# gudbrandtandberg/ChessVision-3LC

Hardware: AMD Instinct MI355X
Metric: boards/sec (UNet 256x256 seg + 64-sq classify) (higher is better)
Workload: dtype f16x3; 1 GPU; e2e-cnn b=256/GPU: UNet(3->1,convT) 256x256 x256 boards + ResNet-18(1ch,13cls) x16384 squares/step; in HBM (configs[3]); boards_per_gpu=256, parallelism=replicas x1, boards sharded, weights RCCL-broadcast once

## Files before the change

chessvision-3lc_amd/csrc/conv_device.h:

```cpp
#pragma once
#include <type_traits>

#include "cv_kernels.h"

namespace cv {

#ifndef CV_STAMP
#define CV_STAMP 0
#endif
#ifndef CV_IGEMM_PIPE
#define CV_IGEMM_PIPE 1
#endif
#ifndef CV_SCHED_HINTS
#define CV_SCHED_HINTS 1
#endif
#ifndef CV_SETPRIO
#define CV_SETPRIO 1
#endif
constexpr bool kSetPrio = CV_SETPRIO != 0;
#ifndef CV_ABLATE
#define CV_ABLATE 0
#endif

template <typename T> struct FragT;
template <> struct FragT<half_t> { typedef half8 V; };
template <> struct FragT<float>  { typedef f4 V; };
template <> struct FragT<split_t> { typedef half8 V; };

__device__ __forceinline__ void mma16(f4& acc, const half8& a, const half8& b) {
#if CV_ABLATE == 2
    asm volatile("" ::"v"(a), "v"(b));
#else
    acc = __builtin_amdgcn_mfma_f32_16x16x32_f16(a, b, acc, 0, 0, 0);
#endif
}
__device__ __forceinline__ void mma16(f4& acc, const f4& a, const f4& b) {
    acc = __builtin_amdgcn_mfma_f32_16x16x4f32(a[0], b[0], acc, 0, 0, 0);
    acc = __builtin_amdgcn_mfma_f32_16x16x4f32(a[1], b[1], acc, 0, 0, 0);
    acc = __builtin_amdgcn_mfma_f32_16x16x4f32(a[2], b[2], acc, 0, 0, 0);
    acc = __builtin_amdgcn_mfma_f32_16x16x4f32(a[3], b[3], acc, 0, 0, 0);
}

__device__ __forceinline__ void glds16(const char* g, char* l) {
    __builtin_amdgcn_global_load_lds((const __attribute__((address_space(1))) void*)g,
                                     (__attribute__((address_space(3))) void*)l, 16, 0, 0);
}

__device__ __forceinline__ void glds16s(const char* sbase, unsigned voff, char* l) {
    __builtin_amdgcn_global_load_lds((const __attribute__((address_space(1))) void*)(sbase + voff),
                                     (__attribute__((address_space(3))) void*)l, 16, 0, 0);
}

template <int N> __device__ __forceinline__ void wait_vm_barrier() {
    asm volatile("s_waitcnt vmcnt(%0) lgkmcnt(0)\n\ts_barrier" ::"n"(N) : "memory");
}

template <typename T, int N> struct OutVec;
template <int N> struct OutVec<half_t, N> {
    static __device__ __forceinline__ void store(half_t* dst, int, const float* v, float& bad) {
#pragma unroll
        for (int i = 0; i < N; i += 8) {
            half8 h;
#pragma unroll
            for (int j = 0; j < 8; ++j) { h[j] = (half_t)v[i + j]; bad = __builtin_fmaf((float)h[j], 0.f, bad); }
            *reinterpret_cast<half8*>(dst + i) = h;
        }
    }
    static constexpr int kRawChunks = N / 8;
    static __device__ __forceinline__ void fetch(const half_t* src, f4* raw) {
#pragma unroll
        for (int i = 0; i < N / 8; ++i) raw[i] = *reinterpret_cast<const f4*>(src + i * 8);
    }
    static __device__ __forceinline__ void add_raw(const f4* raw, int, float* v, float mul) {
#pragma unroll
        for (int i = 0; i < N; i += 8) {
            const half8 h = __builtin_bit_cast(half8, raw[i / 8]);
#pragma unroll
            for (int j = 0; j < 8; ++j) v[i + j] = __builtin_fmaf((float)h[j], mul, v[i + j]);
        }
    }
    static __device__ __forceinline__ void add(const half_t* src, int, float* v, float mul) {
#pragma unroll
        for (int i = 0; i < N; i += 8) {
            const half8 h = *reinterpret_cast<const half8*>(src + i);
#pragma unroll
            for (int j = 0; j < 8; ++j) v[i + j] = __builtin_fmaf((float)h[j], mul, v[i + j]);
        }
    }
};
template <int N> struct OutVec<float, N> {
    static __device__ __forceinline__ void store(float* dst, int, const float* v, float& bad) {
#pragma unroll
        for (int i = 0; i < N; i += 4) {
            f4 o = {v[i], v[i + 1], v[i + 2], v[i + 3]};
#pragma unroll
            for (int j = 0; j < 4; ++j) bad = __builtin_fmaf(o[j], 0.f, bad);
            *reinterpret_cast<f4*>(dst + i) = o;
        }
    }
    static constexpr int kRawChunks = N / 4;
    static __device__ __forceinline__ void fetch(const float* src, f4* raw) {
#pragma unroll
        for (int i = 0; i < N / 4; ++i) raw[i] = *reinterpret_cast<const f4*>(src + i * 4);
    }
    static __device__ __forceinline__ void add_raw(const f4* raw, int, float* v, float) {
#pragma unroll
        for (int i = 0; i < N; i += 4) { v[i] += raw[i / 4][0]; v[i + 1] += raw[i / 4][1]; v[i + 2] += raw[i / 4][2]; v[i + 3] += raw[i / 4][3]; }
    }
    static __device__ __forceinline__ void add(const float* src, int, float* v, float) {
#pragma unroll
        for (int i = 0; i < N; i += 4) {
            const f4 o = *reinterpret_cast<const f4*>(src + i);
            v[i] += o[0]; v[i + 1] += o[1]; v[i + 2] += o[2]; v[i + 3] += o[3];
        }
    }
};
template <int N> struct OutVec<split_t, N> {
    static __device__ __forceinline__ void store(split_t* dst, int ch0, const float* v, float& bad) {
        char* p = reinterpret_cast<char*>(dst);
#pragma unroll
        for (int i = 0; i < N; i += 8) {
            const int par = ((ch0 + i) >> 3) & 1;
            typedef _Float16 h2 __attribute__((ext_vector_type(2)));
            typedef unsigned u4 __attribute__((ext_vector_type(4)));
            u4 hu, lu;
            h2 g2 = {(half_t)0.f, (half_t)0.f};
#pragma unroll
            for (int j = 0; j < 8; j += 2) {
                unsigned hp, lp;
                split_pair(v[i + j], v[i + j + 1], hp, lp);
                g2 = __builtin_elementwise_fma(__builtin_bit_cast(h2, hp), h2{(half_t)0.f, (half_t)0.f}, g2);
                hu[j / 2] = hp; lu[j / 2] = lp;
            }
// ... 65 lines not shown
```

chessvision-3lc_amd/csrc/conv_halo.hip:

```cpp
#include "cv_kernels.h"
#include "conv_igemm.h"
#include "conv_device.h"

#include <cstdlib>

namespace cv {

constexpr int kHaloCT = 64, kHaloNW = 4, kHaloNSW = 3;
constexpr int halo_waves_per_eu(int chain) { return chain == 1 ? 1 : 2; }
template <typename T, int TH, int IMG, bool PERSIST, bool FUSE0 = false, int CHAIN = 0, int CNB = 2>
__global__ __launch_bounds__(64 * kHaloNW) __attribute__((amdgpu_waves_per_eu(halo_waves_per_eu(CHAIN), halo_waves_per_eu(CHAIN)))) void conv3x3_halo_kernel(const ConvParams p) {
    constexpr int CT = kHaloCT, NW = kHaloNW, NSW = kHaloNSW;
    constexpr bool DBH = TH == 8;
    static_assert(CT == 64 && NSW == 3, "every wave owns a 64-channel slab; the ring slot of a stage is tap % 3");
    static_assert(TH == 16 || (TH == 8 && IMG == 0 && !PERSIST), "16 x 16 patch with one halo buffer | 8 x 16 patch, double buffered");
    static_assert(!FUSE0 || (!DBH && !PERSIST && IMG == 0 && __is_same(T, split_t)), "fused producer: split-f16 64-channel single-halo tile");
    static_assert(!CHAIN || (!DBH && !PERSIST && !FUSE0 && IMG == 0 && __is_same(T, half_t)), "chained convolutions: f16 64-channel single-halo tile over whole 16 x 16 images");
    static_assert(CNB == 2 || (CHAIN && CNB == 3), "two or three chained BasicBlocks");
    constexpr int SPC = 9;
    constexpr int FC = 4;
    constexpr int FP = TH / NW;
    static_assert(FP >= 1 && FP <= 4 && TH % NW == 0, "wave tile");
    constexpr int WSTAGE = CT * 128;
    static_assert(IMG == 0 || (IMG == 8 && TH == 16), "packed-image mode: 2 x 2 images of 8 x 8");
    constexpr int HLW = IMG ? IMG + 2 : 18;
    constexpr int HR = IMG ? 4 * HLW * HLW : 18 * (TH + 2);
    constexpr int H = ((HR + 7) / 8 + NW - 1) / NW;
    constexpr int HBYTES = H * NW * 1024;
    constexpr int LW = CT / (8 * NW);
    static_assert(LW >= 1 && LW + H <= 63, "vmcnt range");
    constexpr bool kSplit16 = sizeof(T) == 4 && !__is_same(T, float);
    typedef typename FragT<T>::V V;

    extern __shared__ __attribute__((aligned(16))) char smem[];
    char* const halo = smem + NSW * WSTAGE;
#if CV_STAMP
    const unsigned long long st_k0 = __builtin_amdgcn_s_memtime();
#endif

    const int tid = threadIdx.x;
    const int lane = tid & 63;
    const int wave = __builtin_amdgcn_readfirstlane(tid >> 6);
    const unsigned nwg = gridDim.x, bid = blockIdx.x;
    const unsigned xq = nwg >> 3, xr = nwg & 7, xcd = bid & 7;
    const unsigned lid = (xcd < xr ? xcd * (xq + 1) : xr * (xq + 1) + (xcd - xr) * xq) + (bid >> 3);
    const int tilesX = IMG ? 1 : p.Wo / 16, tilesY = IMG ? 1 : p.Ho / TH;
    const int nImg = p.M / (p.Ho * p.Wo);
    const int kSplits = (!PERSIST && !FUSE0 && IMG == 0 && p.ksplit > 1) ? p.ksplit : 1;
    const int nCbAll = p.nStages / 9;
    int nCb = nCbAll, nS = nCb * SPC, cbBase = 0, ksCur = 0;
    const unsigned nTiles = (unsigned)((IMG ? (nImg + 3) / 4 : nImg * tilesX * tilesY) * p.nCt);
    int ctTile, tx, ty, n;
    unsigned hbase;
    const char* wsrc;
    unsigned hoff[H];

    const unsigned xpix = (unsigned)p.xCs * (unsigned)sizeof(T);
    const char* const xsrc = p.x + p.xCoffBytes;
    const int wi = wave;
    const unsigned lane16 = (unsigned)lane * 16u;
    auto halo_row_offset = [&](int i) __attribute__((always_inline)) -> unsigned {
        const int r = (i * NW + wi) * 8 + (lane >> 3);
        const int rr = r < HR ? r : HR - 1;
        if constexpr (IMG == 0) {
            const int hy = rr / 18, hx = rr - hy * 18;
            return (hbase + (unsigned)(hy * p.xWp + hx)) * xpix + (unsigned)(((lane & 7) ^ (hx & 7)) * 16);
        } else {
            const int lim = (nImg - n) * (HLW * HLW) - 1;
            const int rc = rr < lim ? rr : lim;
            const int hx = (rr % (HLW * HLW)) % HLW;
            return (unsigned)(n * (HLW * HLW) + rc) * xpix + (unsigned)(((lane & 7) ^ (hx & 7)) * 16);
        }
    };
    auto decode = [&](unsigned tile) __attribute__((always_inline)) {
        int pt;
        if (kSplits > 1) {
            const int nPatch = nImg * tilesX * tilesY;
            pt = tile % nPatch;
            const int rest = tile / nPatch;
            ctTile = rest % p.nCt;
            ksCur = rest / p.nCt;
            cbBase = ksCur * p.kper;
            nCb = nCbAll - cbBase < p.kper ? nCbAll - cbBase : p.kper;
            nS = nCb * SPC;
        } else {
            ctTile = tile % p.nCt;
            pt = tile / p.nCt;
        }
        tx = pt % tilesX; pt /= tilesX;
        ty = pt % tilesY;
        n = IMG ? 4 * (pt / tilesY) : pt / tilesY;
        hbase = (unsigned)((n * p.xHp + ty * TH) * p.xWp + tx * 16);
        wsrc = p.w + ((size_t)ctTile * p.nStages + (size_t)cbBase * 9) * WSTAGE + wi * 1024;
#pragma unroll
        for (int i = 0; i < H; ++i) hoff[i] = halo_row_offset(i);
    };

    const int q = lane >> 4, l15 = lane & 15;
    auto issue_w = [&](int s, int slot) __attribute__((always_inline)) {
        char* sW = smem + slot * WSTAGE;
#pragma unroll
        for (int i = 0; i < LW; ++i) glds16s(wsrc + (size_t)s * WSTAGE + i * (NW * 1024), lane16, sW + (i * NW + wi) * 1024);
    };
    auto issue_halo = [&](int cb, int hb) __attribute__((always_inline)) {
        char* sH = halo + hb * HBYTES;
        const char* const src = xsrc + (cbBase + cb) * 128;
#pragma unroll
        for (int i = 0; i < H; ++i) glds16s(src, hoff[i], sH + (i * NW + wi) * 1024);
    };

    constexpr int PW0 = 20;
    unsigned* const patch0 = reinterpret_cast<unsigned*>(halo + HBYTES);
    half8* const w0lds = reinterpret_cast<half8*>(halo + HBYTES + 4864);
    float* const sc0lds = reinterpret_cast<float*>(halo + HBYTES + 4864 + 4096);
    auto load_patch0 = [&]() __attribute__((always_inline)) {
        w0lds[tid] = reinterpret_cast<const half8*>(p.f0_w)[2 * 2 * 64 + tid];
        if (tid < 64) { sc0lds[tid] = p.f0_scale[tid]; sc0lds[64 + tid] = p.f0_shift[tid]; }
        float bad0 = 0.f;
        for (int idx = tid; idx < 3 * 20 * PW0 + 1; idx += 64 * NW) {
            const int c = idx / (20 * PW0), rem = idx - c * (20 * PW0), r = rem / PW0, col = rem - r * PW0;
            const int gy = ty * TH - 2 + r, gx = tx * 16 - 2 + col;
            float v = 0.f;
            if (idx < 3 * 20 * PW0 && gy >= 0 && gy < p.xHp - 2 && gx >= 0 && gx < p.xWp - 2) {
                const int Hh = p.xHp - 2, Ww = p.xWp - 2;
                if (p.f0_u8) v = (float)reinterpret_cast<const uint8_t*>(p.f0_x)[((size_t)(n * Hh + gy) * Ww + gx) * 3 + c] / 255.f;
                else v = reinterpret_cast<const float*>(p.f0_x)[((size_t)(n * 3 + c) * Hh + gy) * Ww + gx];
            }
            bad0 = __builtin_fmaf(v, 0.f, bad0);
            v *= p.f0_in_mul;
            const half_t vh = (half_t)v;
            const half_t vl = (half_t)(v - (float)vh);
            patch0[idx] = (unsigned)__builtin_bit_cast(unsigned short, vh) | ((unsigned)__builtin_bit_cast(unsigned short, vl) << 16);
        }
        if (bad0 != bad0 && p.flag) atomicMin(p.flag, 0u);
    };
    auto produce0 = [&](int cb) __attribute__((always_inline)) {
        half8 ah0, al0, ah1, al1;
        if (cb == 0) {
            const half8* w0 = reinterpret_cast<const half8*>(p.f0_w) + lane;
            ah0 = w0[0 * 64]; al0 = w0[1 * 64]; ah1 = w0[2 * 64]; al1 = w0[3 * 64];
        } else {
            ah0 = w0lds[0 * 64 + lane]; al0 = w0lds[1 * 64 + lane]; ah1 = w0lds[2 * 64 + lane]; al1 = w0lds[3 * 64 + lane];
        }
        float sc0[8], sh0[8];
#pragma unroll
        for (int j = 0; j < 8; j += 4) {
            const f4 a = *reinterpret_cast<const f4*>(sc0lds + cb * 32 + q * 8 + j);
            const f4 b = *reinterpret_cast<const f4*>(sc0lds + 64 + cb * 32 + q * 8 + j);
            sc0[j] = a[0]; sc0[j + 1] = a[1]; sc0[j + 2] = a[2]; sc0[j + 3] = a[3];
            sh0[j] = b[0]; sh0[j + 1] = b[1]; sh0[j + 2] = b[2]; sh0[j + 3] = b[3];
        }
        int ko[8];
#pragma unroll
        for (int j = 0; j < 8; ++j) {
            const int k = q * 8 + j, tap = k / 3, c = k - tap * 3, ky = tap / 3, kx = tap - ky * 3;
            ko[j] = k < 27 ? (c * 20 + ky) * PW0 + kx : 3 * 20 * PW0;
        }
        constexpr int NF = (HR + 15) / 16, U = 3;
        typedef unsigned u4 __attribute__((ext_vector_type(4)));
        int hp = wave * 16 + l15;
        int hy = hp / 18, hx = hp - hy * 18;
        for (int fr0 = wave; fr0 < NF; fr0 += U * NW) {
            int hyu[U], hxu[U], hpu[U];
            unsigned w8[U][8];
#pragma unroll
            for (int u = 0; u < U; ++u) {
                hpu[u] = hp;
                const bool tail = hp >= HR;
                hyu[u] = tail ? 17 : hy; hxu[u] = tail ? 17 : hx;
                const int pb = hyu[u] * PW0 + hxu[u];
#pragma unroll
                for (int j = 0; j < 8; ++j) w8[u][j] = patch0[(q * 8 + j < 27 ? pb : 0) + ko[j]];
                hp += 16 * NW;
                hx += (16 * NW) % 18; hy += (16 * NW) / 18;
                if (hx >= 18) { hx -= 18; hy += 1; }
            }
            f4 a0[U], a1[U];
            half8 bh[U], bl[U];
#pragma unroll
            for (int u = 0; u < U; ++u) {
                u4 uh, ul;
#pragma unroll
                for (int m = 0; m < 4; ++m) {
                    uh[m] = __builtin_amdgcn_perm(w8[u][2 * m + 1], w8[u][2 * m], 0x05040100u);
                    ul[m] = __builtin_amdgcn_perm(w8[u][2 * m + 1], w8[u][2 * m], 0x07060302u);
                }
                bh[u] = __builtin_bit_cast(half8, uh); bl[u] = __builtin_bit_cast(half8, ul);
            }
#pragma unroll
            for (int u = 0; u < U; ++u) {
                a0[u] = __builtin_amdgcn_mfma_f32_16x16x32_f16(ah0, bh[u], f4{0.f, 0.f, 0.f, 0.f}, 0, 0, 0);
                a1[u] = __builtin_amdgcn_mfma_f32_16x16x32_f16(ah1, bh[u], f4{0.f, 0.f, 0.f, 0.f}, 0, 0, 0);
            }
#pragma unroll
            for (int u = 0; u < U; ++u) {
                a0[u] = __builtin_amdgcn_mfma_f32_16x16x32_f16(al0, bh[u], a0[u], 0, 0, 0);
                a1[u] = __builtin_amdgcn_mfma_f32_16x16x32_f16(al1, bh[u], a1[u], 0, 0, 0);
// ... 108 lines not shown
#pragma unroll
                for (int f = 0; f < 4; ++f) rtrunk[g][f] = *reinterpret_cast<const f4*>(rb + (size_t)(pix0 + (unsigned)(g * p.yWp)) * 64 + f * 4);
        }
    };
    auto chain_epilogue = [&](int c) __attribute__((always_inline)) {
        if constexpr (CHAIN) {
            const bool has_res = (c & 1) != 0, last = c == 2 * CNB - 1;
            const int blk = c >> 1;
            const float* const scp = p.ch_scale[c] + q * 16;
            const float* const shp = p.ch_shift[c] + q * 16;
            float sc[16], sh[16];
#pragma unroll
            for (int i = 0; i < 16; i += 4) {
                const f4 a = *reinterpret_cast<const f4*>(scp + i);
                const f4 b = *reinterpret_cast<const f4*>(shp + i);
                sc[i] = a[0]; sc[i + 1] = a[1]; sc[i + 2] = a[2]; sc[i + 3] = a[3];
                sh[i] = b[0]; sh[i + 1] = b[1]; sh[i + 2] = b[2]; sh[i + 3] = b[3];
            }
            const unsigned pix0 = (unsigned)((n * p.yHp + wrow0 + 1) * p.yWp + l15 + 1);
            f4 r[2][4];
            const float* const rb = reinterpret_cast<const float*>(blk == 0 ? p.ch_res0 : p.ch_y32_mid[blk - 1]) + q * 16;
            auto fetch_res = [&](int g) __attribute__((always_inline)) {
#pragma unroll
                for (int f = 0; f < 4; ++f) r[g & 1][f] = *reinterpret_cast<const f4*>(rb + (size_t)(pix0 + (unsigned)(g * p.yWp)) * 64 + f * 4);
            };
            if (CHAIN == 2 && has_res) fetch_res(0);
            const float rm = p.ch_res_mul[blk];
            float* const o32 = reinterpret_cast<float*>(has_res && !last ? p.ch_y32_mid[blk] : p.y32) + q * 16;
            half_t* const o16 = reinterpret_cast<half_t*>(p.y) + q * 16;
            const int hx = l15 + 1;
            float bad = 0.f;
#pragma unroll
            for (int g = 0; g < FP; ++g) {
                if (CHAIN == 2 && has_res && g + 1 < FP) fetch_res(g + 1);
                float v[16];
#pragma unroll
                for (int f = 0; f < 4; ++f)
#pragma unroll
                    for (int k = 0; k < 4; ++k) {
                        float t = acc[f][g][k] * sc[f * 4 + k] + sh[f * 4 + k];
                        if constexpr (CHAIN == 2) {
                            if (has_res) t = __builtin_fmaf(r[g & 1][f][k], rm, t);
                        } else {
                            if (has_res) t = __builtin_fmaf(rtrunk[g][f][k], rm, t);
                        }
                        v[f * 4 + k] = __builtin_fmaxf(t, 0.f);
                        if constexpr (CHAIN == 1) {
                            if (has_res) rtrunk[g][f][k] = v[f * 4 + k];
                        }
                    }
                half8 h0, h1;
#pragma unroll
                for (int j = 0; j < 8; ++j) {
                    h0[j] = (half_t)v[j]; h1[j] = (half_t)v[8 + j];
                    bad = __builtin_fmaf((float)h0[j], 0.f, bad); bad = __builtin_fmaf((float)h1[j], 0.f, bad);
                }
                const size_t pix = (size_t)(pix0 + (unsigned)(g * p.yWp));
                if (has_res && (CHAIN == 2 || last)) {
#pragma unroll
                    for (int f = 0; f < 4; ++f) *reinterpret_cast<f4*>(o32 + pix * 64 + f * 4) = f4{v[f * 4], v[f * 4 + 1], v[f * 4 + 2], v[f * 4 + 3]};
                }
                if (last) {
                    *reinterpret_cast<half8*>(o16 + pix * 64) = h0;
                    *reinterpret_cast<half8*>(o16 + pix * 64 + 8) = h1;
                } else {
                    char* const row = halo + ((wrow0 + g + 1) * 18 + hx) * 128;
                    *reinterpret_cast<half8*>(row + (((2 * q) ^ (hx & 7)) << 4)) = h0;
                    *reinterpret_cast<half8*>(row + (((2 * q + 1) ^ (hx & 7)) << 4)) = h1;
                }
            }
            if (bad != bad && p.flag) atomicMin(p.flag, p.ch_layer_id[c]);
        }
    };

    Frags F0, F1;
    int s = 0;
    auto issue_prologue_halo = [&]() __attribute__((always_inline)) {
        if (!FUSE0) issue_halo(0, 0);
    };
    auto issue_prologue_w = [&]() __attribute__((always_inline)) {
        issue_w(0, 0); issue_w(1, 1); issue_w(2, 2);
    };
    auto issue_prologue = [&]() __attribute__((always_inline)) {
        issue_prologue_halo();
        issue_prologue_w();
    };
    auto stage = [&](Frags& cur, Frags& nxt, auto j_tag, auto hb_tag, int cb) __attribute__((always_inline)) {
        constexpr int J = decltype(j_tag)::value;
        constexpr int HB = decltype(hb_tag)::value;
        const bool more_cb = cb + 1 < nCb;
        constexpr bool kRefill = !DBH && J == 8;
        constexpr bool kRefillIssue = !DBH && J == 7;
#if CV_STAMP
        const unsigned long long st_0 = __builtin_amdgcn_s_memtime();
#endif
        __builtin_amdgcn_sched_barrier(0);
#if CV_ABLATE != 3
        if constexpr (!kRefill)
            load_b(nxt, std::integral_constant<int, (J + 1) % 9>{}, std::integral_constant<int, (DBH && J == 8 ? HB ^ 1 : HB)>{});
#endif
        mma_head(cur);
#if CV_SCHED_HINTS
        __builtin_amdgcn_sched_group_barrier(0x008, kMfmaPerMma, 0);
#pragma unroll
        for (int i = 0; i < 2 * FP; ++i) {
            __builtin_amdgcn_sched_group_barrier(0x100, 1, 0);
            __builtin_amdgcn_sched_group_barrier(0x008, kMfmaPerMma, 0);
        }
#endif
        const bool halo_young = !FUSE0 && !CHAIN && more_cb && (DBH ? (J >= 1 && J <= NSW - 1) : J == 8);
        const bool chain_young = CHAIN == 2 && J <= 1 && cb >= 2 && (cb & 1) == 0;
#if CV_STAMP
        const unsigned long long st_a = __builtin_amdgcn_s_memtime();
#endif
        __builtin_amdgcn_sched_barrier(0);
        constexpr int FLY = (NSW - 2) * LW;
        static_assert(FLY + H <= 63, "vmcnt range");
        if (halo_young) wait_vm_barrier<FLY + H>();
        else if (chain_young) wait_vm_barrier<FLY + kChainStores>();
        else wait_vm_barrier<FLY>();
        __builtin_amdgcn_sched_barrier(0);
#if CV_STAMP
        const unsigned long long st_b = __builtin_amdgcn_s_memtime();
#endif
#if CV_ABLATE != 1 && CV_ABLATE != 3
        issue_w(s + NSW < nS ? s + NSW : nS - 1, J % 3);
        if (kRefillIssue && !FUSE0 && !CHAIN && more_cb) issue_halo(cb + 1, 0);
        if (DBH && J == 0 && more_cb) issue_halo(cb + 1, HB ^ 1);
#endif
#if CV_ABLATE != 3
        load_a(nxt, std::integral_constant<int, (J + 1) % 3>{});
#endif
#if CV_STAMP
        const unsigned long long st_c = __builtin_amdgcn_s_memtime();
#endif
        mma_tail(cur);
#if CV_SCHED_HINTS
#pragma unroll
        for (int i = 0; i < LW + (kRefillIssue && !FUSE0 && !CHAIN ? H : 0); ++i) {
            __builtin_amdgcn_sched_group_barrier(0x020, 1, 0);
            __builtin_amdgcn_sched_group_barrier(0x008, 1, 0);
        }
#pragma unroll
        for (int i = 0; i < 2 * FC; ++i) {
            __builtin_amdgcn_sched_group_barrier(0x100, 1, 0);
            __builtin_amdgcn_sched_group_barrier(0x008, MPL, 0);
        }
#endif
        if constexpr (kRefill) {
            if (more_cb) {
                __builtin_amdgcn_sched_barrier(0);
                if constexpr (FUSE0) {
                    produce0(cb + 1);
                    asm volatile("s_waitcnt lgkmcnt(0)\n\ts_barrier" ::: "memory");
                } else if constexpr (CHAIN) {
                    chain_epilogue(cb);
#pragma unroll
                    for (int f = 0; f < FC; ++f)
#pragma unroll
                        for (int g = 0; g < FP; ++g) acc[f][g] = f4{0.f, 0.f, 0.f, 0.f};
                    asm volatile("s_waitcnt lgkmcnt(0)\n\ts_barrier" ::: "memory");
                } else {
                    asm volatile("s_waitcnt vmcnt(%0)\n\ts_barrier" ::"n"(LW) : "memory");
                }
                load_b(nxt, std::integral_constant<int, 0>{}, std::integral_constant<int, 0>{});
                __builtin_amdgcn_sched_barrier(0);
            }
        }
#if CV_STAMP
        const unsigned long long st_d = __builtin_amdgcn_s_memtime();
        st_head += st_a - st_0; st_wait += st_b - st_a; st_tail += st_d - st_b; (void)st_c;
#endif
        ++s;
    };
    auto run_cb = [&](auto pb_tag, int cb) __attribute__((always_inline)) {
        constexpr int PB = decltype(pb_tag)::value;
        typedef std::integral_constant<int, DBH ? PB : 0> HBt;
        Frags& E = PB ? F1 : F0;
        Frags& O = PB ? F0 : F1;
        stage(E, O, std::integral_constant<int, 0>{}, HBt{}, cb); stage(O, E, std::integral_constant<int, 1>{}, HBt{}, cb);
        stage(E, O, std::integral_constant<int, 2>{}, HBt{}, cb); stage(O, E, std::integral_constant<int, 3>{}, HBt{}, cb);
        stage(E, O, std::integral_constant<int, 4>{}, HBt{}, cb); stage(O, E, std::integral_constant<int, 5>{}, HBt{}, cb);
        stage(E, O, std::integral_constant<int, 6>{}, HBt{}, cb); stage(O, E, std::integral_constant<int, 7>{}, HBt{}, cb);
        stage(E, O, std::integral_constant<int, 8>{}, HBt{}, cb);
    };
    unsigned tile = lid;
    decode(tile);
    issue_prologue();
    chain_load_trunk();
    if constexpr (FUSE0) {
        load_patch0();
        asm volatile("s_waitcnt lgkmcnt(0)\n\ts_barrier" ::: "memory");
        produce0(0);
        asm volatile("s_waitcnt lgkmcnt(0)\n\ts_barrier" ::: "memory");
    }
    for (bool first = true;; first = false) {
#pragma unroll
    for (int f = 0; f < FC; ++f)
#pragma unroll
        for (int g = 0; g < FP; ++g) acc[f][g] = f4{0.f, 0.f, 0.f, 0.f};
    if (first) {
        wait_vm_barrier<(NSW - 1) * LW>();
    } else {
        wait_vm_barrier<0>();
    }
    load_a(F0, std::integral_constant<int, 0>{});
    load_b(F0, std::integral_constant<int, 0>{}, std::integral_constant<int, 0>{});
    s = 0;
    for (int cb = 0; cb < nCb; cb += 2) {
        run_cb(std::integral_constant<int, 0>{}, cb);
        if (cb + 1 < nCb) run_cb(std::integral_constant<int, 1>{}, cb + 1);
    }
    asm volatile("s_waitcnt vmcnt(0)" ::: "memory");

#if CV_STAMP
    const unsigned long long st_t1 = __builtin_amdgcn_s_memtime(), st_r1 = __builtin_amdgcn_s_memrealtime();
    if (p.stamp && lane == 0) {
        unsigned long long* o = p.stamp + ((size_t)bid * NW + wave) * 8;
        o[0] = st_t1 - st_t0; o[1] = st_r1 - st_r0; o[2] = st_wait; o[3] = (unsigned long long)nS;
        o[4] = st_head; o[5] = st_t0 - st_k0; o[6] = st_tail;
    }
#endif
    if constexpr (CHAIN == 1) {
        chain_epilogue(2 * CNB - 1);
        return;
    }
    const int eCt = ctTile, eTx = tx, eTy = ty, eN = n;
    const unsigned nxt_tile = tile + nwg;
    const bool more_tiles = PERSIST && nxt_tile < nTiles;
    constexpr int NV = 4 * FC;
    const int row0 = eCt * CT + wci * 64 + q * NV;
    float sc[NV], sh[NV];
#pragma unroll
    for (int i = 0; i < NV; i += 4) {
        const f4 a = *reinterpret_cast<const f4*>(p.scale + row0 + i);
        const f4 b = *reinterpret_cast<const f4*>(p.shift + row0 + i);
        sc[i] = a[0]; sc[i + 1] = a[1]; sc[i + 2] = a[2]; sc[i + 3] = a[3];
        sh[i] = b[0]; sh[i + 1] = b[1]; sh[i + 2] = b[2]; sh[i + 3] = b[3];
    }
    if (kSplits > 1) {
        float* const part = p.partial + (size_t)ksCur * p.M * p.prow + row0;
#pragma unroll
        for (int g = 0; g < FP; ++g) {
            const size_t pix = ((size_t)eN * p.Ho + eTy * TH + wrow0 + g) * p.Wo + eTx * 16 + l15;
#pragma unroll
            for (int f = 0; f < FC; ++f) *reinterpret_cast<f4*>(part + pix * p.prow + f * 4) = acc[f][g];
        }
        return;
    }
    T* const ybase = reinterpret_cast<T*>(p.y);
    const T* const rbase = reinterpret_cast<const T*>(p.res);
    const int oimg = IMG ? eN + (wrow0 >> 3) * 2 + (l15 >> 3) : eN;
    const int oy0 = IMG ? (wrow0 & 7) : eTy * TH + wrow0, ox = IMG ? (l15 & 7) : eTx * 16 + l15;

    if (!PERSIST && p.head_w) {
        float hw[NV];
#pragma unroll
        for (int i = 0; i < NV; ++i) hw[i] = p.head_w[row0 + i];
#pragma unroll
        for (int g = 0; g < FP; ++g) {
            float part = 0.f;
#pragma unroll
            for (int f = 0; f < FC; ++f)
#pragma unroll
                for (int r = 0; r < 4; ++r) {
                    float v = acc[f][g][r] * sc[f * 4 + r] + sh[f * 4 + r];
                    v = (p.relu && v < 0.f) ? 0.f : v;
                    part = __builtin_fmaf(v, hw[f * 4 + r], part);
                }
            part += __shfl_xor(part, 16);
            part += __shfl_xor(part, 32);
            if (q == 0) {
                const size_t pix = ((size_t)oimg * p.Ho + oy0 + g) * p.Wo + ox;
                const float l = part + p.head_b[0];
                p.head_logits[pix] = l;
                if (p.head_mask) p.head_mask[pix] = (1.f / (1.f + __expf(-l))) > p.head_thr ? 255 : 0;
                report_bad(p, l * 0.f);
            }
        }
#if CV_STAMP
        asm volatile("s_waitcnt vmcnt(0)" ::: "memory");
        if (p.stamp && lane == 0) p.stamp[((size_t)bid * NW + wave) * 8 + 7] = __builtin_amdgcn_s_memtime() - st_t1;
#endif
        return;
    }

    constexpr int UN = __is_same(T, float) ? 4 : 8;
    constexpr int UPP = 64 / UN;
    constexpr int UPL = 16 * UPP / 64;
    constexpr int SROW = 272;
    asm volatile("s_waitcnt lgkmcnt(0)\n\ts_barrier" ::: "memory");
#if CV_STAMP
    const unsigned long long st_e0 = __builtin_amdgcn_s_memtime();
#endif
    if (more_tiles) {
        decode(nxt_tile);
        issue_prologue_halo();
    }
    constexpr int RG = PERSIST ? 1 : 2;
    static_assert(FP % 2 == 0 && NW * RG * 16 * SROW <= (PERSIST ? NSW * WSTAGE : NSW * WSTAGE + (DBH ? 2 : 1) * HBYTES), "staging must fit in LDS");
    char* const stg = smem + wave * (RG * 16 * SROW);
    const int slab0 = eCt * CT + wci * 64;
    T* const pbase = reinterpret_cast<T*>(p.pool_y);
    const bool relu_early = p.relu && !rbase;
    auto out_pixel = [&](int g, int px, bool* live) __attribute__((always_inline)) -> unsigned {
        if constexpr (IMG == 0) {
            *live = true;
            return (unsigned)((eN * p.yHp + oy0 + g + 1) * p.yWp + eTx * 16 + px + 1);
        } else {
            const int img = eN + (wrow0 >> 3) * 2 + (px >> 3);
            *live = img < nImg;
            return (unsigned)((img * p.yHp + oy0 + g + 1) * p.yWp + (px & 7) + 1);
        }
    };
    float hold[UPL][UN];
    constexpr bool kHalf = __is_same(T, half_t);
    constexpr int RC = kHalf ? 2 : OutVec<T, UN>::kRawChunks;
    constexpr bool kPrefetchRes = !PERSIST;
    const bool res32 = kHalf && p.res_f32;
    const float* const rbase32 = reinterpret_cast<const float*>(p.res);
    float* const ybase32 = kHalf ? reinterpret_cast<float*>(p.y32) : nullptr;
    f4 rraw[kPrefetchRes ? FP : 1][UPL][RC];
    if constexpr (kPrefetchRes) {
        if (rbase) {
#pragma unroll
            for (int g = 0; g < FP; ++g)
#pragma unroll
                for (int i = 0; i < UPL; ++i) {
                    const int unit = lane + 64 * i, px = unit / UPP, co = slab0 + (unit % UPP) * UN;
                    bool live;
                    const unsigned ob = out_pixel(g, px, &live);
                    if (co < p.rows && live) {
                        if (res32) trunk32_fetch(rbase32 + (ob * (unsigned)p.rCs + (unsigned)(p.rCoff + co)), rraw[g][i]);
                        else OutVec<T, UN>::fetch(rbase + (ob * (unsigned)p.rCs + (unsigned)(p.rCoff + co)), rraw[g][i]);
                    } else {
#pragma unroll
                        for (int c = 0; c < RC; ++c) rraw[g][i][c] = f4{0.f, 0.f, 0.f, 0.f};
                    }
                }
        }
    }
    float bad = 0.f;
#pragma unroll
    for (int g0 = 0; g0 < FP; g0 += RG) {
#pragma unroll
        for (int r = 0; r < RG; ++r)
#pragma unroll
            for (int f = 0; f < FC; ++f) {
                f4 t;
#pragma unroll
                for (int k = 0; k < 4; ++k) {
                    t[k] = acc[f][g0 + r][k] * sc[f * 4 + k] + sh[f * 4 + k];
                    if (relu_early) t[k] = __builtin_fmaxf(t[k], 0.f);
                }
                *reinterpret_cast<f4*>(stg + r * (16 * SROW) + l15 * SROW + (q * NV + f * 4) * 4) = t;
            }
        wave_lds_sync();
#pragma unroll
        for (int i = 0; i < UPL; ++i) {
            const int unit = lane + 64 * i;
            const int px = unit / UPP, cu = unit % UPP;
            const int co = slab0 + cu * UN;
            float w[RG][UN];
#pragma unroll
            for (int r = 0; r < RG; ++r)
#pragma unroll
                for (int j = 0; j < UN; j += 4) {
                    const f4 t = *reinterpret_cast<const f4*>(stg + r * (16 * SROW) + px * SROW + (cu * UN + j) * 4);
                    w[r][j] = t[0]; w[r][j + 1] = t[1]; w[r][j + 2] = t[2]; w[r][j + 3] = t[3];
                }
#pragma unroll
            for (int r = 0; r < RG; ++r) {
                bool live;
                const unsigned ob = out_pixel(g0 + r, px, &live);
                if (co < p.rows && live) {
                    if (rbase) {
                        if (res32) {
                            if constexpr (kHalf) {
                                if constexpr (kPrefetchRes) trunk32_add_raw(rraw[g0 + r][i], w[r], p.res_mul);
                                else {
                                    f4 raw[2];
                                    trunk32_fetch(rbase32 + (ob * (unsigned)p.rCs + (unsigned)(p.rCoff + co)), raw);
                                    trunk32_add_raw(raw, w[r], p.res_mul);
                                }
                            }
                        } else if constexpr (kPrefetchRes) OutVec<T, UN>::add_raw(rraw[g0 + r][i], p.rCoff + co, w[r], p.res_mul);
                        else OutVec<T, UN>::add(rbase + (ob * (unsigned)p.rCs + (unsigned)(p.rCoff + co)), p.rCoff + co, w[r], p.res_mul);
                        if (p.relu) {
#pragma unroll
                            for (int j = 0; j < UN; ++j) w[r][j] = __builtin_fmaxf(w[r][j], 0.f);
                        }
                    }
                    OutVec<T, UN>::store(ybase + (ob * (unsigned)p.yCs + (unsigned)(p.yCoff + co)), p.yCoff + co, w[r], bad);
                    if constexpr (kHalf) {
                        if (ybase32) trunk32_store(ybase32 + (ob * (unsigned)p.yCs + (unsigned)(p.yCoff + co)), w[r]);
                    }
                }
            }
            if (IMG == 0 && pbase) {
                float m[UN];
#pragma unroll
                for (int j = 0; j < UN; j += 4) {
                    f4 best = *reinterpret_cast<const f4*>(stg + (px ^ 1) * SROW + (cu * UN + j) * 4);
#pragma unroll
                    for (int r = 1; r < RG; ++r) {
                        const f4 t = *reinterpret_cast<const f4*>(stg + r * (16 * SROW) + (px ^ 1) * SROW + (cu * UN + j) * 4);
#pragma unroll
                        for (int k = 0; k < 4; ++k) best[k] = best[k] > t[k] ? best[k] : t[k];
                    }
#pragma unroll
                    for (int k = 0; k < 4; ++k) {
                        float v = w[0][j + k];
#pragma unroll
                        for (int r = 1; r < RG; ++r) v = v > w[r][j + k] ? v : w[r][j + k];
                        m[j + k] = v > best[k] ? v : best[k];
                    }
                }
                bool emit = true;
                if constexpr (RG == 1) {
                    if ((g0 & 1) == 0) {
                        emit = false;
#pragma unroll
                        for (int j = 0; j < UN; ++j) hold[i][j] = m[j];
                    } else {
#pragma unroll
                        for (int j = 0; j < UN; ++j) m[j] = m[j] > hold[i][j] ? m[j] : hold[i][j];
                    }
                }
                const unsigned qb = (unsigned)((eN * p.pHp + ((oy0 + g0) >> 1) + 1) * p.pWp + ((eTx * 16 + px) >> 1) + 1);
                if constexpr (kSplit16) {
                    if (emit && co < p.rows)
                        OutVec<T, UN>::store_half(pbase + (qb * (unsigned)p.pCs + (unsigned)(p.pCoff + co)), p.pCoff + co, m, (px & 1) == 0);
                } else {
                    if (emit && (px & 1) == 0 && co < p.rows)
                        OutVec<T, UN>::store(pbase + (qb * (unsigned)p.pCs + (unsigned)(p.pCoff + co)), p.pCoff + co, m, bad);
                }
            }
        }
        wave_lds_sync();
    }
#if CV_STAMP
    const unsigned long long st_e1 = __builtin_amdgcn_s_memtime();
    asm volatile("s_waitcnt vmcnt(0)" ::: "memory");
    if (p.stamp && lane == 0) {
        unsigned long long* o = p.stamp + ((size_t)bid * NW + wave) * 8;
        o[7] = __builtin_amdgcn_s_memtime() - st_t1;
        o[4] = st_e0 - st_t1;
        o[6] = st_e1 - st_t1;
    }
#endif
    report_bad(p, bad);
    if (!more_tiles) break;
    if constexpr (PERSIST) {
        asm volatile("s_waitcnt lgkmcnt(0)\n\ts_barrier" ::: "memory");
        issue_prologue_w();
    }
    tile = nxt_tile;
    }
}

template <int TH, int IMG>
static constexpr size_t halo_lds() {
    constexpr int HR = IMG ? 4 * (IMG + 2) * (IMG + 2) : 18 * (TH + 2);
    constexpr int H = ((HR + 7) / 8 + kHaloNW - 1) / kHaloNW;
    return (size_t)kHaloNSW * kHaloCT * 128 + (size_t)(TH == 8 ? 2 : 1) * H * kHaloNW * 1024;
}

static int g_halo_cus = 256;

constexpr size_t kFuse0Lds = 4864 + 4096 + 512;
template <typename T, int TH, int IMG> static constexpr bool halo_can_fuse0() { return TH == 16 && IMG == 0 && __is_same(T, split_t); }

template <typename T, int TH, int IMG>
static hipError_t launch_halo(const ConvParams& p, int n_images, hipStream_t stream) {
    const bool split = p.ksplit > 1;
    if (split && (IMG != 0 || p.f0_x || !p.partial || p.kper < 1)) return hipErrorInvalidValue;
    const int tiles = (IMG ? (n_images + 3) / 4 : n_images * (p.Ho / TH) * (p.Wo / 16)) * p.nCt * (split ? p.ksplit : 1);
    const size_t lds = halo_lds<TH, IMG>();
    if (p.f0_x) {
        if constexpr (halo_can_fuse0<T, TH, IMG>()) {
            auto kern = conv3x3_halo_kernel<T, TH, IMG, false, true>;
            hipLaunchKernelGGL(kern, dim3((unsigned)tiles), dim3(64 * kHaloNW), lds + kFuse0Lds, stream, p);
            return hipGetLastError();
        } else {
            return hipErrorInvalidValue;
        }
    }
    static_assert(halo_lds<TH, IMG>() <= 160 * 1024, "LDS budget");
    if constexpr (TH == 16 && IMG == 0) {
        static const int on64 = [] { const char* v = std::getenv("CV_HALO_PERSIST64"); return v && *v ? std::atoi(v) : 0; }();
        static const int max_k64 = [] { const char* v = std::getenv("CV_HALO_PERSIST64_MAXK"); return v && *v ? std::atoi(v) : 36; }();
        if (on64 && !split && !p.head_w && !p.res && tiles >= 8 * g_halo_cus && p.nStages <= max_k64) {
            auto kern = conv3x3_halo_kernel<T, TH, IMG, true>;
            hipLaunchKernelGGL(kern, dim3((unsigned)(2 * g_halo_cus)), dim3(64 * kHaloNW), lds, stream, p);
            return hipGetLastError();
        }
    }
    auto kern = conv3x3_halo_kernel<T, TH, IMG, false>;
    hipLaunchKernelGGL(kern, dim3((unsigned)tiles), dim3(64 * kHaloNW), lds, stream, p);
    return hipGetLastError();
}

static hipError_t halo_allow_lds(void (*kern)(const ConvParams)) {
    return hipFuncSetAttribute(reinterpret_cast<const void*>(kern), hipFuncAttributeMaxDynamicSharedMemorySize, 160 * 1024);
}

template <typename T, int TH, int IMG>
static hipError_t prepare_halo() {
    hipError_t e = halo_allow_lds(conv3x3_halo_kernel<T, TH, IMG, false>);
    if constexpr (halo_can_fuse0<T, TH, IMG>()) {
        if (e == hipSuccess) e = halo_allow_lds(conv3x3_halo_kernel<T, TH, IMG, false, true>);
    }
    if constexpr (TH == 16 && IMG == 0) {
        if (e == hipSuccess) e = halo_allow_lds(conv3x3_halo_kernel<T, TH, IMG, true>);
    }
    return e;
}

#define CV_FOR_EACH_HALO(X, T) X(T, 16, 0) X(T, 16, 8) X(T, 8, 0)

static void (*const kChainKernels[2][2])(const ConvParams) = {
    {conv3x3_halo_kernel<half_t, 16, 0, false, false, 1, 2>, conv3x3_halo_kernel<half_t, 16, 0, false, false, 1, 3>},
    {conv3x3_halo_kernel<half_t, 16, 0, false, false, 2, 2>, conv3x3_halo_kernel<half_t, 16, 0, false, false, 2, 3>}};

hipError_t conv_halo_prepare() {
    hipError_t e;
    int dev = 0, cus = 0;
    if (hipGetDevice(&dev) == hipSuccess && hipDeviceGetAttribute(&cus, hipDeviceAttributeMultiprocessorCount, dev) == hipSuccess && cus > 0)
        g_halo_cus = cus;
#define X(T, TH, IMG) \
    if ((e = prepare_halo<T, TH, IMG>()) != hipSuccess) return e;
    CV_FOR_EACH_HALO(X, half_t)
    CV_FOR_EACH_HALO(X, float)
    CV_FOR_EACH_HALO(X, split_t)
#undef X
    for (const auto& form : kChainKernels)
        for (const auto kern : form)
            if ((e = halo_allow_lds(kern)) != hipSuccess) return e;
    return hipSuccess;
}

bool conv_halo_can_fuse_first_layer(int dt) { return dt == kSplit; }

bool conv_halo_supported(int Ho, int Wo) {
    static const bool allow_img8 = [] { const char* v = std::getenv("CV_HALO_IMG8"); return !(v && v[0] == '0'); }();
    if (Ho == 8 && Wo == 8) return allow_img8;
    return Ho % 16 == 0 && Wo % 16 == 0;
}

hipError_t conv_halo_chain_launch(const ConvParams& p, int n_images, hipStream_t stream) {
    if (!p.chain || (p.nStages != 36 && p.nStages != 54) || p.Ho != 16 || p.Wo != 16 || p.yCs != 64 || p.xCs != 64 || p.ksplit > 1 || n_images < 1)
        return hipErrorInvalidValue;
    const size_t lds = halo_lds<16, 0>();
// ... 17 lines not shown
```

Baseline: 4093 boards/sec.

## Prefetch BN scale/shift and head weights into LDS; specialize epilogue by residual/pool mode

Per-tile scale, shift and head weight/bias vectors are now loaded asynchronously into a small LDS region with global_load_lds during the prologue, instead of being read from global memory in the epilogue. The store epilogue is also turned into a lambda instantiated per residual/pool mode, so runtime branches on rbase, res32 and pbase become compile-time constants. This aims to hide epilogue load latency and remove branch overhead, at the cost of extra LDS, a static assert limiting occupancy to two workgroups per CU, and larger code.

```diff
diff --git a/chessvision-3lc_amd/csrc/conv_device.h b/chessvision-3lc_amd/csrc/conv_device.h
--- a/chessvision-3lc_amd/csrc/conv_device.h
+++ b/chessvision-3lc_amd/csrc/conv_device.h
@@ -49,6 +49,11 @@
 __device__ __forceinline__ void glds16s(const char* sbase, unsigned voff, char* l) {
     __builtin_amdgcn_global_load_lds((const __attribute__((address_space(1))) void*)(sbase + voff),
                                      (__attribute__((address_space(3))) void*)l, 16, 0, 0);
+}
+
+__device__ __forceinline__ void glds4(const float* g, float* l) {
+    __builtin_amdgcn_global_load_lds((const __attribute__((address_space(1))) void*)g,
+                                     (__attribute__((address_space(3))) void*)l, 4, 0, 0);
 }
 
 template <int N> __device__ __forceinline__ void wait_vm_barrier() {
diff --git a/chessvision-3lc_amd/csrc/conv_halo.hip b/chessvision-3lc_amd/csrc/conv_halo.hip
--- a/chessvision-3lc_amd/csrc/conv_halo.hip
+++ b/chessvision-3lc_amd/csrc/conv_halo.hip
@@ -7,6 +7,8 @@
 namespace cv {
 
 constexpr int kHaloCT = 64, kHaloNW = 4, kHaloNSW = 3;
+constexpr int kHaloCstLds = 4 * 64 * 4;
+constexpr int kFuse0Lds = 4864 + 4096 + 512;
 constexpr int halo_waves_per_eu(int chain) { return chain == 1 ? 1 : 2; }
 template <typename T, int TH, int IMG, bool PERSIST, bool FUSE0 = false, int CHAIN = 0, int CNB = 2>
 __global__ __launch_bounds__(64 * kHaloNW) __attribute__((amdgpu_waves_per_eu(halo_waves_per_eu(CHAIN), halo_waves_per_eu(CHAIN)))) void conv3x3_halo_kernel(const ConvParams p) {
@@ -113,6 +115,16 @@
     unsigned* const patch0 = reinterpret_cast<unsigned*>(halo + HBYTES);
     half8* const w0lds = reinterpret_cast<half8*>(halo + HBYTES + 4864);
     float* const sc0lds = reinterpret_cast<float*>(halo + HBYTES + 4864 + 4096);
+    static_assert(!FUSE0 || 4864 + 4096 + 512 == kFuse0Lds, "fused producer tables");
+    static_assert(NSW * WSTAGE + (DBH ? 2 : 1) * HBYTES + (FUSE0 ? kFuse0Lds : 0) + kHaloCstLds <= 80 * 1024, "two workgroups per CU");
+    float* const cst = reinterpret_cast<float*>(halo + (DBH ? 2 : 1) * HBYTES + (FUSE0 ? kFuse0Lds : 0));
+    constexpr bool kHead = !PERSIST && !CHAIN;
+    auto issue_consts = [&]() __attribute__((always_inline)) {
+        if constexpr (CHAIN != 1) {
+            if (wave < 2) glds4((wave ? p.shift : p.scale) + ctTile * CT + lane, cst + wave * 64);
+            else if (kHead && p.head_w) glds4(wave == 2 ? p.head_w + lane : p.head_b, cst + wave * 64);
+        }
+    };
     auto load_patch0 = [&]() __attribute__((always_inline)) {
         w0lds[tid] = reinterpret_cast<const half8*>(p.f0_w)[2 * 2 * 64 + tid];
         if (tid < 64) { sc0lds[tid] = p.f0_scale[tid]; sc0lds[64 + tid] = p.f0_shift[tid]; }
@@ -387,6 +399,7 @@
         issue_w(0, 0); issue_w(1, 1); issue_w(2, 2);
     };
     auto issue_prologue = [&]() __attribute__((always_inline)) {
+        issue_consts();
         issue_prologue_halo();
         issue_prologue_w();
     };
@@ -538,8 +551,8 @@
     float sc[NV], sh[NV];
 #pragma unroll
     for (int i = 0; i < NV; i += 4) {
-        const f4 a = *reinterpret_cast<const f4*>(p.scale + row0 + i);
-        const f4 b = *reinterpret_cast<const f4*>(p.shift + row0 + i);
+        const f4 a = *reinterpret_cast<const f4*>(cst + q * NV + i);
+        const f4 b = *reinterpret_cast<const f4*>(cst + 64 + q * NV + i);
         sc[i] = a[0]; sc[i + 1] = a[1]; sc[i + 2] = a[2]; sc[i + 3] = a[3];
         sh[i] = b[0]; sh[i + 1] = b[1]; sh[i + 2] = b[2]; sh[i + 3] = b[3];
     }
@@ -558,10 +571,14 @@
     const int oimg = IMG ? eN + (wrow0 >> 3) * 2 + (l15 >> 3) : eN;
     const int oy0 = IMG ? (wrow0 & 7) : eTy * TH + wrow0, ox = IMG ? (l15 & 7) : eTx * 16 + l15;
 
-    if (!PERSIST && p.head_w) {
+    if (kHead && p.head_w) {
         float hw[NV];
 #pragma unroll
-        for (int i = 0; i < NV; ++i) hw[i] = p.head_w[row0 + i];
+        for (int i = 0; i < NV; i += 4) {
+            const f4 a = *reinterpret_cast<const f4*>(cst + 128 + q * NV + i);
+            hw[i] = a[0]; hw[i + 1] = a[1]; hw[i + 2] = a[2]; hw[i + 3] = a[3];
+        }
+        const float head_b = cst[192];
 #pragma unroll
         for (int g = 0; g < FP; ++g) {
             float part = 0.f;
@@ -577,7 +594,7 @@
             part += __shfl_xor(part, 32);
             if (q == 0) {
                 const size_t pix = ((size_t)oimg * p.Ho + oy0 + g) * p.Wo + ox;
-                const float l = part + p.head_b[0];
+                const float l = part + head_b;
                 p.head_logits[pix] = l;
                 if (p.head_mask) p.head_mask[pix] = (1.f / (1.f + __expf(-l))) > p.head_thr ? 255 : 0;
                 report_bad(p, l * 0.f);
@@ -600,6 +617,7 @@
 #endif
     if (more_tiles) {
         decode(nxt_tile);
+        issue_consts();
         issue_prologue_halo();
     }
     constexpr int RG = PERSIST ? 1 : 2;
@@ -607,7 +625,6 @@
     char* const stg = smem + wave * (RG * 16 * SROW);
     const int slab0 = eCt * CT + wci * 64;
     T* const pbase = reinterpret_cast<T*>(p.pool_y);
-    const bool relu_early = p.relu && !rbase;
     auto out_pixel = [&](int g, int px, bool* live) __attribute__((always_inline)) -> unsigned {
         if constexpr (IMG == 0) {
             *live = true;
@@ -628,122 +645,136 @@
     f4 rraw[kPrefetchRes ? FP : 1][UPL][RC];
     if constexpr (kPrefetchRes) {
         if (rbase) {
-#pragma unroll
-            for (int g = 0; g < FP; ++g)
-#pragma unroll
-                for (int i = 0; i < UPL; ++i) {
-                    const int unit = lane + 64 * i, px = unit / UPP, co = slab0 + (unit % UPP) * UN;
+            auto res_offset = [&](int g, int i) __attribute__((always_inline)) -> unsigned {
+                const int unit = lane + 64 * i, px = unit / UPP, co = slab0 + (unit % UPP) * UN;
+                bool live;
+                const unsigned ob = out_pixel(g, px, &live);
+                return (co < p.rows && live) ? ob * (unsigned)p.rCs + (unsigned)(p.rCoff + co) : (unsigned)p.rCoff;
+            };
+            if (res32) {
+#pragma unroll
+                for (int g = 0; g < FP; ++g)
+#pragma unroll
+                    for (int i = 0; i < UPL; ++i) trunk32_fetch(rbase32 + res_offset(g, i), rraw[g][i]);
+            } else {
+#pragma unroll
+                for (int g = 0; g < FP; ++g)
+#pragma unroll
+                    for (int i = 0; i < UPL; ++i) OutVec<T, UN>::fetch(rbase + res_offset(g, i), rraw[g][i]);
+            }
+        }
+    }
+    float bad = 0.f;
+    auto store_rows = [&](auto res_tag, auto pool_tag) __attribute__((always_inline)) {
+        constexpr int RES = decltype(res_tag)::value;
+        constexpr int POOL = decltype(pool_tag)::value;
+        const bool relu_early = p.relu && RES == 0;
+#pragma unroll
+        for (int g0 = 0; g0 < FP; g0 += RG) {
+#pragma unroll
+            for (int r = 0; r < RG; ++r)
+#pragma unroll
+                for (int f = 0; f < FC; ++f) {
+                    f4 t;
+#pragma unroll
+                    for (int k = 0; k < 4; ++k) {
+                        t[k] = acc[f][g0 + r][k] * sc[f * 4 + k] + sh[f * 4 + k];
+                        if (relu_early) t[k] = __builtin_fmaxf(t[k], 0.f);
+                    }
+                    *reinterpret_cast<f4*>(stg + r * (16 * SROW) + l15 * SROW + (q * NV + f * 4) * 4) = t;
+                }
+            wave_lds_sync();
+#pragma unroll
+            for (int i = 0; i < UPL; ++i) {
+                const int unit = lane + 64 * i;
+                const int px = unit / UPP, cu = unit % UPP;
+                const int co = slab0 + cu * UN;
+                float w[RG][UN];
+#pragma unroll
+                for (int r = 0; r < RG; ++r)
+#pragma unroll
+                    for (int j = 0; j < UN; j += 4) {
+                        const f4 t = *reinterpret_cast<const f4*>(stg + r * (16 * SROW) + px * SROW + (cu * UN + j) * 4);
+                        w[r][j] = t[0]; w[r][j + 1] = t[1]; w[r][j + 2] = t[2]; w[r][j + 3] = t[3];
+                    }
+#pragma unroll
+                for (int r = 0; r < RG; ++r) {
                     bool live;
-                    const unsigned ob = out_pixel(g, px, &live);
+                    const unsigned ob = out_pixel(g0 + r, px, &live);
                     if (co < p.rows && live) {
-                        if (res32) trunk32_fetch(rbase32 + (ob * (unsigned)p.rCs + (unsigned)(p.rCoff + co)), rraw[g][i]);
-                        else OutVec<T, UN>::fetch(rbase + (ob * (unsigned)p.rCs + (unsigned)(p.rCoff + co)), rraw[g][i]);
-                    } else {
-#pragma unroll
-                        for (int c = 0; c < RC; ++c) rraw[g][i][c] = f4{0.f, 0.f, 0.f, 0.f};
-                    }
-                }
-        }
-    }
-    float bad = 0.f;
-#pragma unroll
-    for (int g0 = 0; g0 < FP; g0 += RG) {
-#pragma unroll
-        for (int r = 0; r < RG; ++r)
-#pragma unroll
-            for (int f = 0; f < FC; ++f) {
-                f4 t;
-#pragma unroll
-                for (int k = 0; k < 4; ++k) {
-                    t[k] = acc[f][g0 + r][k] * sc[f * 4 + k] + sh[f * 4 + k];
-                    if (relu_early) t[k] = __builtin_fmaxf(t[k], 0.f);
-                }
-                *reinterpret_cast<f4*>(stg + r * (16 * SROW) + l15 * SROW + (q * NV + f * 4) * 4) = t;
-            }
-        wave_lds_sync();
-#pragma unroll
-        for (int i = 0; i < UPL; ++i) {
-            const int unit = lane + 64 * i;
-            const int px = unit / UPP, cu = unit % UPP;
-            const int co = slab0 + cu * UN;
-            float w[RG][UN];
-#pragma unroll
-            for (int r = 0; r < RG; ++r)
-#pragma unroll
-                for (int j = 0; j < UN; j += 4) {
-                    const f4 t = *reinterpret_cast<const f4*>(stg + r * (16 * SROW) + px * SROW + (cu * UN + j) * 4);
-                    w[r][j] = t[0]; w[r][j + 1] = t[1]; w[r][j + 2] = t[2]; w[r][j + 3] = t[3];
-                }
-#pragma unroll
-            for (int r = 0; r < RG; ++r) {
-                bool live;
-                const unsigned ob = out_pixel(g0 + r, px, &live);
-                if (co < p.rows && live) {
-                    if (rbase) {
-                        if (res32) {
-                            if constexpr (kHalf) {
-                                if constexpr (kPrefetchRes) trunk32_add_raw(rraw[g0 + r][i], w[r], p.res_mul);
-                                else {
-                                    f4 raw[2];
-                                    trunk32_fetch(rbase32 + (ob * (unsigned)p.rCs + (unsigned)(p.rCoff + co)), raw);
-                                    trunk32_add_raw(raw, w[r], p.res_mul);
+                        if constexpr (RES != 0) {
+                            if constexpr (RES == 2) {
+                                if constexpr (kHalf) {
+                                    if constexpr (kPrefetchRes) trunk32_add_raw(rraw[g0 + r][i], w[r], p.res_mul);
+                                    else {
+                                        f4 raw[2];
+                                        trunk32_fetch(rbase32 + (ob * (unsigned)p.rCs + (unsigned)(p.rCoff + co)), raw);
+                                        trunk32_add_raw(raw, w[r], p.res_mul);
+                                    }
                                 }
+                            } else if constexpr (kPrefetchRes) OutVec<T, UN>::add_raw(rraw[g0 + r][i], p.rCoff + co, w[r], p.res_mul);
+                            else OutVec<T, UN>::add(rbase + (ob * (unsigned)p.rCs + (unsigned)(p.rCoff + co)), p.rCoff + co, w[r], p.res_mul);
+                            if (p.relu) {
+#pragma unroll
+                                for (int j = 0; j < UN; ++j) w[r][j] = __builtin_fmaxf(w[r][j], 0.f);
                             }
-                        } else if constexpr (kPrefetchRes) OutVec<T, UN>::add_raw(rraw[g0 + r][i], p.rCoff + co, w[r], p.res_mul);
-                        else OutVec<T, UN>::add(rbase + (ob * (unsigned)p.rCs + (unsigned)(p.rCoff + co)), p.rCoff + co, w[r], p.res_mul);
-                        if (p.relu) {
-#pragma unroll
-                            for (int j = 0; j < UN; ++j) w[r][j] = __builtin_fmaxf(w[r][j], 0.f);
+                        }
+                        OutVec<T, UN>::store(ybase + (ob * (unsigned)p.yCs + (unsigned)(p.yCoff + co)), p.yCoff + co, w[r], bad);
+                        if constexpr (kHalf) {
+                            if (ybase32) trunk32_store(ybase32 + (ob * (unsigned)p.yCs + (unsigned)(p.yCoff + co)), w[r]);
                         }
                     }
-                    OutVec<T, UN>::store(ybase + (ob * (unsigned)p.yCs + (unsigned)(p.yCoff + co)), p.yCoff + co, w[r], bad);
-                    if constexpr (kHalf) {
-                        if (ybase32) trunk32_store(ybase32 + (ob * (unsigned)p.yCs + (unsigned)(p.yCoff + co)), w[r]);
+                }
+                if (IMG == 0 && (POOL == 1 || (POOL == 2 && pbase))) {
+                    float m[UN];
+#pragma unroll
+                    for (int j = 0; j < UN; j += 4) {
+                        f4 best = *reinterpret_cast<const f4*>(stg + (px ^ 1) * SROW + (cu * UN + j) * 4);
+#pragma unroll
+                        for (int r = 1; r < RG; ++r) {
+                            const f4 t = *reinterpret_cast<const f4*>(stg + r * (16 * SROW) + (px ^ 1) * SROW + (cu * UN + j) * 4);
+#pragma unroll
+                            for (int k = 0; k < 4; ++k) best[k] = best[k] > t[k] ? best[k] : t[k];
+                        }
+#pragma unroll
+                        for (int k = 0; k < 4; ++k) {
+                            float v = w[0][j + k];
+#pragma unroll
+                            for (int r = 1; r < RG; ++r) v = v > w[r][j + k] ? v : w[r][j + k];
+                            m[j + k] = v > best[k] ? v : best[k];
+                        }
                     }
-                }
-            }
-            if (IMG == 0 && pbase) {
-                float m[UN];
-#pragma unroll
-                for (int j = 0; j < UN; j += 4) {
-                    f4 best = *reinterpret_cast<const f4*>(stg + (px ^ 1) * SROW + (cu * UN + j) * 4);
-#pragma unroll
-                    for (int r = 1; r < RG; ++r) {
-                        const f4 t = *reinterpret_cast<const f4*>(stg + r * (16 * SROW) + (px ^ 1) * SROW + (cu * UN + j) * 4);
-#pragma unroll
-                        for (int k = 0; k < 4; ++k) best[k] = best[k] > t[k] ? best[k] : t[k];
+                    bool emit = true;
+                    if constexpr (RG == 1) {
+                        if ((g0 & 1) == 0) {
+                            emit = false;
+#pragma unroll
+                            for (int j = 0; j < UN; ++j) hold[i][j] = m[j];
+                        } else {
+#pragma unroll
+                            for (int j = 0; j < UN; ++j) m[j] = m[j] > hold[i][j] ? m[j] : hold[i][j];
+                        }
                     }
-#pragma unroll
-                    for (int k = 0; k < 4; ++k) {
-                        float v = w[0][j + k];
-#pragma unroll
-                        for (int r = 1; r < RG; ++r) v = v > w[r][j + k] ? v : w[r][j + k];
-                        m[j + k] = v > best[k] ? v : best[k];
+                    const unsigned qb = (unsigned)((eN * p.pHp + ((oy0 + g0) >> 1) + 1) * p.pWp + ((eTx * 16 + px) >> 1) + 1);
+                    if constexpr (kSplit16) {
+                        if (emit && co < p.rows)
+                            OutVec<T, UN>::store_half(pbase + (qb * (unsigned)p.pCs + (unsigned)(p.pCoff + co)), p.pCoff + co, m, (px & 1) == 0);
+                    } else {
+                        if (emit && (px & 1) == 0 && co < p.rows)
+                            OutVec<T, UN>::store(pbase + (qb * (unsigned)p.pCs + (unsigned)(p.pCoff + co)), p.pCoff + co, m, bad);
                     }
                 }
-                bool emit = true;
-                if constexpr (RG == 1) {
-                    if ((g0 & 1) == 0) {
-                        emit = false;
-#pragma unroll
-                        for (int j = 0; j < UN; ++j) hold[i][j] = m[j];
-                    } else {
-#pragma unroll
-                        for (int j = 0; j < UN; ++j) m[j] = m[j] > hold[i][j] ? m[j] : hold[i][j];
-                    }
-                }
-                const unsigned qb = (unsigned)((eN * p.pHp + ((oy0 + g0) >> 1) + 1) * p.pWp + ((eTx * 16 + px) >> 1) + 1);
-                if constexpr (kSplit16) {
-                    if (emit && co < p.rows)
-                        OutVec<T, UN>::store_half(pbase + (qb * (unsigned)p.pCs + (unsigned)(p.pCoff + co)), p.pCoff + co, m, (px & 1) == 0);
-                } else {
-                    if (emit && (px & 1) == 0 && co < p.rows)
-                        OutVec<T, UN>::store(pbase + (qb * (unsigned)p.pCs + (unsigned)(p.pCoff + co)), p.pCoff + co, m, bad);
-                }
-            }
-        }
-        wave_lds_sync();
-    }
+            }
+            wave_lds_sync();
+        }
+    };
+    typedef std::integral_constant<int, 0> tag0;
+    typedef std::integral_constant<int, 1> tag1;
+    typedef std::integral_constant<int, 2> tag2;
+    if (rbase && res32) store_rows(tag2{}, tag2{});
+    else if (rbase) store_rows(tag1{}, tag2{});
+    else if (IMG == 0 && pbase) store_rows(tag0{}, tag1{});
+    else store_rows(tag0{}, tag0{});
 #if CV_STAMP
     const unsigned long long st_e1 = __builtin_amdgcn_s_memtime();
     asm volatile("s_waitcnt vmcnt(0)" ::: "memory");
@@ -768,12 +799,11 @@
 static constexpr size_t halo_lds() {
     constexpr int HR = IMG ? 4 * (IMG + 2) * (IMG + 2) : 18 * (TH + 2);
     constexpr int H = ((HR + 7) / 8 + kHaloNW - 1) / kHaloNW;
-    return (size_t)kHaloNSW * kHaloCT * 128 + (size_t)(TH == 8 ? 2 : 1) * H * kHaloNW * 1024;
+    return (size_t)kHaloNSW * kHaloCT * 128 + (size_t)(TH == 8 ? 2 : 1) * H * kHaloNW * 1024 + kHaloCstLds;
 }
 
 static int g_halo_cus = 256;
 
-constexpr size_t kFuse0Lds = 4864 + 4096 + 512;
 template <typename T, int TH, int IMG> static constexpr bool halo_can_fuse0() { return TH == 16 && IMG == 0 && __is_same(T, split_t); }
 
 template <typename T, int TH, int IMG>
```

New measurement: 4107 boards/sec, median of 6. Within noise of the previous version (+0.3%).
